# PoloWlg/Joint-Multimodal-Transformer-6th-ABAW

Measured on AMD Instinct MI355X. Metric: train windows/sec + CCC parity, B=64 T=300 A/V fusion, 1/2/4/8 MI355X, higher is better.
Workload: dtype bf16; 1 GPU; configs[2]: FcLayer(1024,512) + Two_transformers(TRANSFORMER,FC,H=1,L=1,vision_in_ft=2048) + 2x CCCLoss + SGD-nesterov; global_batch=64, per_gpu_batch=64, seq_len=300, D_a=1024, D_v=2048, parallelism=dp1

## Files before the change

### include/jmt.h

```cpp
#ifndef JMT_H_
#define JMT_H_

#include <stddef.h>
#include <stdint.h>

#ifdef __cplusplus
extern "C" {
#endif

#define JMT_ABI_VERSION 7

enum { JMT_F32 = 0, JMT_BF16 = 1, JMT_F16 = 2 };
enum { JMT_OK = 0, JMT_ERR_ARG = -1, JMT_ERR_HIP = -2, JMT_ERR_UNSUPPORTED = -3 };

int jmt_abi_version(void);
const char* jmt_last_error(void);
int jmt_kernel_count(void);
long long jmt_bounds_violations(int reset);

typedef struct jmt_gemm_desc {
  int ab_dtype, c_dtype, aux_dtype;
  int M, N, K;
  const void* a[8];
  const void* b[8];
// ... 58 lines not shown

int jmt_layernorm_fwd_grouped(int dt_in, int dt_out, int G, int64_t rows, int D, const void* x,
                              int64_t ldx, int64_t sx, const void* r, int64_t ldr, int64_t sr,
                              const float* const* gamma, const float* const* beta, float eps,
                              void* y, int64_t ldy, int64_t sy, float* mean, float* rstd,
                              void* stream);
int jmt_layernorm_bwd_grouped(int dt_in, int dt_dy, int dt_dx, int G, int64_t rows, int D,
                              const void* x, int64_t ldx, int64_t sx, const void* r, int64_t ldr,
                              int64_t sr, const void* dy, int64_t lddy, int64_t sdy,
                              const float* mean, const float* rstd, const float* const* gamma,
                              void* dx, int64_t lddx, int64_t sdx, float* const* dgamma,
                              float* const* dbeta, float* const* dsum, int beta_acc,
                              float* partials, void* stream);
int jmt_layernorm_bwd_grouped_blocks(int64_t rows);

int jmt_softmax_fwd(int p_dt, int64_t rows, int n, const float* s, int64_t lds, float scale,
                    void* p, int64_t ldp, void* stream);
int jmt_softmax_bwd(int p_dt, int ds_dt, int64_t rows, int n, const void* p, int64_t ldp,
                    const float* dp, int64_t lddp, float scale, void* ds, int64_t ldds,
                    void* stream);

int jmt_attn_supported(int dt, int dh);
int jmt_attn_fwd(int dt, int N, int H, int Lq, int Lk, int dh, const void* q, int64_t sq_l,
                 int64_t sq_n, const void* k, int64_t sk_l, int64_t sk_n, const void* v,
                 int64_t sv_l, int64_t sv_n, void* o, int64_t so_l, int64_t so_n, float scale,
                 float* lse, void* stream);
int jmt_attn_bwd(int dt, int N, int H, int Lq, int Lk, int dh, const void* go, int64_t sgo_l,
                 int64_t sgo_n, const void* o, int64_t so_l, int64_t so_n, const void* q,
                 int64_t sq_l, int64_t sq_n, const void* k, int64_t sk_l, int64_t sk_n,
                 const void* v, int64_t sv_l, int64_t sv_n, const float* lse, void* p_out,
                 void* ds_out, int64_t ldp, void* dq, int64_t sdq_l, int64_t sdq_n, float scale,
                 void* stream);

int jmt_attn_dkdv(int dt, int N, int H, int Lq, int Lk, int dh, const void* p, const void* ds,
                  int64_t ldp, const void* go, int64_t sgo_l, int64_t sgo_n, const void* q,
                  int64_t sq_l, int64_t sq_n, const void* k, int64_t sk_l, int64_t sk_n, void* dk,
                  int64_t sdk_l, int64_t sdk_n, void* dv, int64_t sdv_l, int64_t sdv_n, void* dq,
                  int64_t sdq_l, int64_t sdq_n, void* stream);

int jmt_attn_short_supported(int dt, int dh, int Lq, int Lk);
int jmt_attn_short_fwd(int dt, int N, int H, int Lq, int Lk, int dh, const void* q, int64_t sq_l,
                       int64_t sq_n, const void* k, int64_t sk_l, int64_t sk_n, const void* v,
                       int64_t sv_l, int64_t sv_n, void* o, int64_t so_l, int64_t so_n,
                       float scale, float* lse, void* stream);
int jmt_attn_short_bwd(int dt, int N, int H, int Lq, int Lk, int dh, const void* go,
                       int64_t sgo_l, int64_t sgo_n, const void* o, int64_t so_l, int64_t so_n,
                       const void* q, int64_t sq_l, int64_t sq_n, const void* k, int64_t sk_l,
                       int64_t sk_n, const void* v, int64_t sv_l, int64_t sv_n, const float* lse,
                       void* dq, int64_t sdq_l, int64_t sdq_n, void* dk, int64_t sdk_l,
                       int64_t sdk_n, void* dv, int64_t sdv_l, int64_t sdv_n, float scale,
                       void* stream);

int jmt_small_attn_fwd(int dt, int N, int H, int Lq, int Lk, int E, const void* q, int64_t sq_l,
                       int64_t sq_n, const void* k, int64_t sk_l, int64_t sk_n, const void* v,
                       int64_t sv_l, int64_t sv_n, void* o, int64_t so_l, int64_t so_n,
                       float scale, float* p_out, void* stream);
int jmt_small_attn_bwd(int dt, int N, int H, int Lq, int Lk, int E, const void* go,
                       int64_t sgo_l, int64_t sgo_n, const void* q, int64_t sq_l, int64_t sq_n,
                       const void* k, int64_t sk_l, int64_t sk_n, const void* v, int64_t sv_l,
                       int64_t sv_n, const float* p, void* dq, int64_t sdq_l, int64_t sdq_n,
                       void* dk, int64_t sdk_l, int64_t sdk_n, void* dv, int64_t sdv_l,
                       int64_t sdv_n, float scale, void* stream);

int jmt_colsum_blocks(int64_t rows);
int jmt_colsum(int dt, int64_t rows, int N, const void* dy, int64_t ld, float* db, int beta_acc,
               float* partials, void* stream);
// ... 86 lines not shown
```

### joint-multimodal-transformer-6th-abaw_amd/csrc/abi_check.cpp

```cpp
#include <stdio.h>
#include <string.h>

#include "../../include/jmt.h"

static int g_fail = 0;

static void expect_msg(const char* what, const char* needle) {
  const char* e = jmt_last_error();
  if (!e || !strstr(e, needle)) {
    fprintf(stderr, "FAIL %s: err='%s' lacks '%s'\n", what, e ? e : "(null)", needle);
    ++g_fail;
  }
}

static void expect_err(const char* what, int rc) {
  const char* e = jmt_last_error();
  const size_t n = e ? strnlen(e, 1024) : 0;
  if (rc >= 0 || n == 0 || n >= 512) {
    fprintf(stderr, "FAIL %s: rc=%d err='%s'\n", what, rc, e ? e : "(null)");
    ++g_fail;
  }
}

int main() {
// ... 93 lines not shown
  }

  expect_err("l2norm_fwd null", jmt_l2norm_fwd(JMT_BF16, JMT_BF16, 8, 512, nullptr, 512, nullptr,
                                               512, fnull, 1e-12f, nullptr));
  expect_err("layernorm_fwd dtype", jmt_layernorm_fwd(9, JMT_BF16, 8, 512, misal, 512, nullptr, 0,
                                                      fnull, fnull, 1e-5f, misal, 512, fnull,
                                                      fnull, nullptr));
  expect_err("softmax_fwd null", jmt_softmax_fwd(JMT_BF16, 8, 300, nullptr, 304, 1.f, nullptr, 304,
                                                 nullptr));
  expect_err("colsum null", jmt_colsum(JMT_BF16, 64, 512, nullptr, 512, fnull, 0, fnull, nullptr));
  expect_err("copy2d dtype", jmt_copy2d(5, 6, 4, 4, misal, 4, 1, misal, 4, 1, 0, nullptr));

  expect_err("attn_fwd head dim", jmt_attn_fwd(JMT_BF16, 2, 1, 300, 300, 64, misal, 512, 512,
                                               misal, 512, 512, misal, 512, 512, misal, 512, 512,
                                               0.1f, fnull, nullptr));
  expect_err("attn_fwd misaligned", jmt_attn_fwd(JMT_BF16, 2, 1, 300, 300, 512, misal, 512, 512,
                                                 misal, 512, 512, misal, 512, 512, misal, 512,
                                                 512, 0.1f, fnull, nullptr));
  expect_err("attn_bwd sizes", jmt_attn_bwd(JMT_BF16, -1, 1, 300, 300, 512, misal, 1, 1, misal, 1,
                                            1, misal, 1, 1, misal, 1, 1, misal, 1, 1, fnull,
                                            misal, misal, 8, misal, 1, 1, 0.1f, nullptr));
  expect_err("attn_dkdv ldp", jmt_attn_dkdv(JMT_BF16, 2, 1, 300, 300, 512, misal, misal, 320,
                                           misal, 512, 512, misal, 512, 512, nullptr, 0, 0,
                                           misal, 512, 512, misal, 512, 512, nullptr, 0, 0,
                                           nullptr));
  expect_err("attn_dkdv head dim", jmt_attn_dkdv(JMT_BF16, 2, 1, 300, 300, 64, misal, misal, 384,
                                                 misal, 512, 512, misal, 512, 512, nullptr, 0, 0,
                                                 misal, 512, 512, misal, 512, 512, nullptr, 0,
                                                 0, nullptr));
  expect_err("attn_dkdv dq misaligned", jmt_attn_dkdv(JMT_BF16, 2, 1, 300, 300, 512, algn, algn,
                                                      384, algn, 512, 512, algn, 512, 512, misal,
                                                      512, 512, algn, 512, 512, algn, 512, 512,
                                                      misal, 512, 512, nullptr));
  expect_err("attn_bwd pds ldp", jmt_attn_bwd(JMT_BF16, 2, 1, 300, 300, 512, algn, 512, 512,
                                              algn, 512, 512, algn, 512, 512, algn, 512, 512,
                                              algn, 512, 512, fnull, algn, algn, 300, nullptr,
                                              0, 0, 0.1f, nullptr));
  expect_err("small_attn_fwd null", jmt_small_attn_fwd(JMT_BF16, 4, 1, 6, 6, 512, nullptr, 512,
                                                       512, nullptr, 512, 512, nullptr, 512, 512,
                                                       nullptr, 512, 512, 0.1f, fnull, nullptr));

  expect_err("ccc_stats kind", jmt_ccc_stats(3, JMT_F32, 10, 1, misal, fnull, 0.f, -1.f, 1.f,
                                             nullptr, nullptr));
  expect_err("ccc_stats bins", jmt_ccc_stats(0, JMT_F32, 10, 100, misal, fnull, 0.f, -1.f, 1.f,
                                             (double*)buf, nullptr));
  expect_err("ccc_finish null", jmt_ccc_finish(0, 0, nullptr, 1, 1e-8f, fnull, nullptr, nullptr));
  expect_err("ccc_finish_add null", jmt_ccc_finish_add(0, 1, nullptr, 1, 1e-8f, fnull, fnull,
                                                       nullptr, nullptr));
  expect_err("ce_stats bins", jmt_ce_stats(JMT_F32, 10, 1, misal, fnull, -1.f, 1.f, fnull,
                                           (double*)buf, nullptr));
  expect_err("ce_bwd null", jmt_ce_bwd(JMT_F32, 10, 5, nullptr, fnull, -1.f, 1.f, fnull, nullptr,
                                       fnull, nullptr, nullptr));
  expect_err("ce_labels null", jmt_ce_labels(10, 5, fnull, -1.f, 1.f, nullptr, nullptr));
  expect_err("mask_indices null", jmt_mask_indices(10, fnull, -5.f, nullptr, nullptr, nullptr));

  expect_err("sgd null", jmt_sgd_step(10, fnull, fnull, fnull, 0.1f, 0.9f, 0.f, 0.f, 1, 1, 1.f,
                                      nullptr, JMT_BF16, nullptr));
  expect_err("sgd_zero null", jmt_sgd_step_zero(10, fnull, nullptr, fnull, 0.1f, 0.9f, 0.f, 0.f,
                                                1, 1, 1.f, nullptr, JMT_BF16, nullptr));
  expect_err("sgd_amp_zero null", jmt_sgd_step_amp_zero(10, fnull, fnull, fnull, 0.1f, 0.9f,
                                                        0.f, 0.f, 1, 1, nullptr, nullptr,
                                                        JMT_BF16, nullptr));
  float* fal = (float*)algn;
  expect_err("opt_tick null state", jmt_opt_tick(nullptr, 0.9, 0.999, nullptr, nullptr));
  expect_msg("opt_tick null state", "null state");
  expect_err("opt_tick beta", jmt_opt_tick(fal, 1.0, 0.999, nullptr, nullptr));
// ... 54 lines not shown
```

### joint-multimodal-transformer-6th-abaw_amd/csrc/attn_dkdv.hip

```cpp
#include "attn_common.h"

namespace jmt {

constexpr int DK_KT = 128;
constexpr int DK_QC = 32;
constexpr int DK_PROW = 2 * DK_KT;
constexpr int DK_IMG = DK_QC * AT_ROWB;
constexpr int DK_PIMG = DK_QC * DK_PROW;
constexpr int DK_STAGE = DK_IMG + DK_PIMG;
#ifndef JMT_DKDV_NS
#define JMT_DKDV_NS 4
#endif
constexpr int DK_NS = JMT_DKDV_NS;
constexpr int DK_LDS = DK_NS * DK_STAGE;
static_assert(DK_NS >= 2 && DK_NS <= 4, "2-4 stages (the wait table covers 0-2 later stages)");
constexpr int DK_NDMA = DK_QC / 8 + 1;
constexpr int DK_NST = 16;

struct AttnDkdvArgs {
  const void* p;
  const void* ds;
  const void* go;
  const void* q;
  const void* k;
  void* dk;
  void* dv;
  void* dq;
  int64_t ldp, sgo_l, sgo_n, sq_l, sq_n, sk_l, sk_n, sdk_l, sdk_n, sdv_l, sdv_n, sdq_l, sdq_n;
  int Lq, Lk, H, nkt, nqd, ipn, nitems;
};

__device__ __forceinline__ int pimg_off(int r, int c) {
  return r * DK_PROW + ((c ^ ((r & 7) << 1)) << 4);
}

__device__ __forceinline__ int qimg_off(int r, int c) {
  return r * 64 + ((c ^ ((r >> 2) & 3)) << 4);
}

struct DkItem {
  int nh, n, hd, role, k0, nch;
};
__device__ __forceinline__ DkItem dk_decode(const AttnDkdvArgs& a, int it) {
  DkItem d;
  d.nh = it / a.ipn;
  const int r = it - d.nh * a.ipn;
  if (r < 2 * a.nkt) {
    d.role = r >= a.nkt;
    d.k0 = (r - d.role * a.nkt) * DK_KT;
    d.nch = (a.Lq + DK_QC - 1) / DK_QC;
  } else {
    d.role = 2;
    d.k0 = (r - 2 * a.nkt) * DK_KT;
    d.nch = (a.Lk + DK_QC - 1) / DK_QC;
  }
  d.n = d.nh / a.H;
  d.hd = d.nh - d.n * a.H;
  return d;
}

template <typename T>
__device__ __forceinline__ void dkdv_stage(char* st, const AttnDkdvArgs& a, const DkItem& d,
                                           int q0) {
  const int lane = threadIdx.x & 63;
  const int wu = __builtin_amdgcn_readfirstlane(threadIdx.x >> 6);
  if (d.role == 2) {
    const char* kb = (const char*)((const T*)a.k + (int64_t)d.n * a.sk_n + d.hd * AT_DH);
    const int ldk = (int)(a.sk_l * (int64_t)sizeof(T));
#pragma unroll
    for (int i = 0; i < DK_QC / 8; ++i) {
      const int r = wu * (DK_QC / 8) + i;
      const int src = min(q0 + r, a.Lk - 1);
      const unsigned off = (unsigned)(lane ^ ((r & 7) << 1)) << 4;
      glds16_asm(kb + (unsigned)(src * ldk) + off, st + r * AT_ROWB);
    }
    const int r = 16 * wu + (lane >> 2);
    const int c = (lane & 3) ^ ((r >> 2) & 3);
    const int src_row = min(d.k0 + r, a.Lq - 1);
    JMT_DCHECK(src_row >= 0 && q0 + 8 * c + 8 <= a.ldp);
    const char* pb = (const char*)((const T*)a.ds + (int64_t)d.nh * a.Lq * a.ldp);
    glds16_asm(pb + (unsigned)(((q0 >> 5) * a.Lq + src_row) * 64) + 16 * c,
               st + DK_IMG + wu * 1024);
    return;
  }
  const char* rb;
  int ldb;
  if (d.role == 0) {
    rb = (const char*)((const T*)a.go + (int64_t)d.n * a.sgo_n + d.hd * AT_DH);
    ldb = (int)(a.sgo_l * (int64_t)sizeof(T));
  } else {
    rb = (const char*)((const T*)a.q + (int64_t)d.n * a.sq_n + d.hd * AT_DH);
    ldb = (int)(a.sq_l * (int64_t)sizeof(T));
  }
#pragma unroll
  for (int i = 0; i < DK_QC / 8; ++i) {
    const int r = wu * (DK_QC / 8) + i;
    const int src = min(q0 + r, a.Lq - 1);
    const unsigned off = (unsigned)(lane ^ ((r & 7) << 1)) << 4;
    glds16_asm(rb + (unsigned)(src * ldb) + off, st + r * AT_ROWB);
  }
  const int r = 4 * wu + (lane >> 4);
  const int cs = (lane & 15) ^ ((r & 7) << 1);
  const int src_row = min(q0 + r, a.Lq - 1);
  JMT_DCHECK(src_row >= 0 && d.k0 + 8 * cs + 8 <= a.ldp);
  if (a.dq) {
    const char* pb = (const char*)((const T*)(d.role == 0 ? a.p : a.ds) +
                                   (int64_t)d.nh * a.Lq * a.ldp);
    glds16_asm(pb + (unsigned)((((d.k0 >> 5) + (cs >> 2)) * a.Lq + src_row) * 64) +
                   16 * (cs & 3),
               st + DK_IMG + wu * 1024);
    return;
  }
  const char* pb = (const char*)((const T*)(d.role == 0 ? a.p : a.ds) +
                                 (int64_t)d.nh * a.Lq * a.ldp + d.k0);
  glds16_asm(pb + (unsigned)(src_row * (int)(a.ldp * sizeof(T))) + 16 * cs,
             st + DK_IMG + wu * 1024);
}

template <int S>
__device__ __forceinline__ void dkdv_wait_s(int stores) {
  switch (stores) {
    case 0: wait_vmcnt<S * DK_NDMA>(); break;
    case 1: wait_vmcnt<S * DK_NDMA + DK_NST>(); break;
    case 2: wait_vmcnt<S * DK_NDMA + 2 * DK_NST>(); break;
    default: wait_vmcnt<S * DK_NDMA + 3 * DK_NST>(); break;
  }
}
__device__ __forceinline__ void dkdv_wait(int stages, int stores) {
  if (stages == 0) dkdv_wait_s<0>(stores);
  else if (stages == 1) dkdv_wait_s<1>(stores);
  else dkdv_wait_s<2>(stores);
}

template <typename T>
__global__ __launch_bounds__(512, 2) void attn_dkdv_kernel(AttnDkdvArgs a) {
  typedef typename Frag16<T>::t F;
  typedef typename Frag16<T>::h Hf;
  typedef unsigned u32x4 __attribute__((ext_vector_type(4)));
  extern __shared__ __attribute__((aligned(16))) char smem[];
  const int lane = threadIdx.x & 63, w = threadIdx.x >> 6;
  const int g = lane >> 4, li = lane & 15;
  int item, iend, istride;
  item_range(a.nitems, item, iend, istride);
  if (item >= iend) return;

  int tb[4], pb[8];
#pragma unroll
  for (int t = 0; t < 4; ++t) tb[t] = tr_base(4 * (w & 1) + t, li, g, 0) + 256 * (w >> 1);
#pragma unroll
  for (int kg = 0; kg < 8; ++kg)
    pb[kg] = pimg_off(4 * g + (li >> 2), 2 * kg + ((li & 3) >> 1)) + 8 * (li & 1);
  const int qb0 = qimg_off(li, g >> 1) + 8 * (g & 1);
  const int qb1 = qimg_off(li, 2 + (g >> 1)) + 8 * (g & 1);

  int is_item = item, is_c = 0;
  DkItem is_d = dk_decode(a, item);
  bool is_ok = true;
  int is_buf = 0;
  unsigned after = 0;
  int inflight = 0;
  auto issue = [&]() {
    if (is_ok) {
      dkdv_stage<T>(smem + is_buf * DK_STAGE, a, is_d, DK_QC * is_c);
      after &= ~(15u << (4 * is_buf));
      ++inflight;
      if (++is_c == is_d.nch) {
        is_c = 0;
        is_item += istride;
        is_ok = is_item < iend;
        if (is_ok) is_d = dk_decode(a, is_item);
      }
    }
    is_buf = is_buf == DK_NS - 1 ? 0 : is_buf + 1;
  };
  for (int i = 0; i < DK_NS - 1; ++i) issue();
  int buf = 0;

  while (true) {
    const DkItem d = dk_decode(a, item);
    const bool more = item + istride < iend;
    f32x4 acc[8][4];
#pragma unroll
    for (int kg = 0; kg < 8; ++kg)
#pragma unroll
      for (int t = 0; t < 4; ++t) acc[kg][t] = f32x4{0.f, 0.f, 0.f, 0.f};

    for (int c = 0; c < d.nch; ++c) {
      const char* cur = smem + buf * DK_STAGE;
      dkdv_wait(inflight - 1, (after >> (4 * buf)) & 15);
      --inflight;
      lds_barrier();
      issue();
      F kf[8];
      const int c0 = DK_QC * c;
      const int clen = d.role == 2 ? a.Lk : a.Lq;
      if (d.role != 2) {
#pragma unroll
        for (int kg = 0; kg < 8; ++kg) {
          const Hf lo = tr_read<Hf>(cur + DK_IMG + pb[kg]);
          const Hf hi = tr_read<Hf>(cur + DK_IMG + pb[kg] + 16 * DK_PROW);
          kf[kg] = __builtin_shufflevector(lo, hi, 0, 1, 2, 3, 4, 5, 6, 7);
        }
      } else {
#pragma unroll
        for (int qg = 0; qg < 8; ++qg) {
          const Hf lo = *(const Hf*)(cur + DK_IMG + qb0 + 1024 * qg);
          const Hf hi = *(const Hf*)(cur + DK_IMG + qb1 + 1024 * qg);
          kf[qg] = __builtin_shufflevector(lo, hi, 0, 1, 2, 3, 4, 5, 6, 7);
        }
      }
      if (c0 + DK_QC > clen) {
#pragma unroll
        for (int e = 0; e < 8; ++e) {
          const bool in = c0 + 16 * (e >> 2) + 4 * g + (e & 3) < clen;
#pragma unroll
          for (int kg = 0; kg < 8; ++kg) kf[kg][e] = in ? kf[kg][e] : from_f<T>(0.f);
        }
      }
      F df[4];
#pragma unroll
      for (int t = 0; t < 4; ++t) {
        const Hf lo = tr_read<Hf>(cur + tb[t]);
        const Hf hi = tr_read<Hf>(cur + tb[t] + 16 * AT_ROWB);
        df[t] = __builtin_shufflevector(lo, hi, 0, 1, 2, 3, 4, 5, 6, 7);
      }
#pragma unroll
      for (int t = 0; t < 4; ++t)
#pragma unroll
        for (int kg = 0; kg < 8; ++kg) acc[kg][t] = mfma16(df[t], kf[kg], acc[kg][t]);
      buf = buf == DK_NS - 1 ? 0 : buf + 1;
    }

    {
      T* ob = d.role == 0 ? (T*)a.dv + (int64_t)d.n * a.sdv_n
            : d.role == 1 ? (T*)a.dk + (int64_t)d.n * a.sdk_n : (T*)a.dq + (int64_t)d.n * a.sdq_n;
      const int64_t sl = d.role == 0 ? a.sdv_l : d.role == 1 ? a.sdk_l : a.sdq_l;
      ob += (int64_t)d.hd * AT_DH + (int64_t)d.k0 * sl;
      const uint64_t ba = (uint64_t)(uintptr_t)ob;
      const uint32_t blo = __builtin_amdgcn_readfirstlane((uint32_t)ba);
      const uint32_t bhi = __builtin_amdgcn_readfirstlane((uint32_t)(ba >> 32));
      const int nrows = min(DK_KT, (d.role == 2 ? a.Lq : a.Lk) - d.k0);
      const int bytes = __builtin_amdgcn_readfirstlane((int)(nrows * sl * (int64_t)sizeof(T)));
      const auto rsrc = __builtin_amdgcn_make_buffer_rsrc(
          (void*)(((uint64_t)bhi << 32) | blo), 0, bytes, 0x00020000);
      const int sl32 = (int)sl;
#pragma unroll
      for (int kg = 0; kg < 8; ++kg) {
#pragma unroll
        for (int jp = 0; jp < 2; ++jp) {
          uint32_t pk[2][2];
#pragma unroll
          for (int hh = 0; hh < 2; ++hh)
#pragma unroll
            for (int qq = 0; qq < 2; ++qq) {
              T two[2] = {from_f<T>(acc[kg][2 * jp + hh][2 * qq]),
                          from_f<T>(acc[kg][2 * jp + hh][2 * qq + 1])};
              pk[hh][qq] = *(const uint32_t*)two;
            }
          const auto r0 = __builtin_amdgcn_permlane16_swap(pk[0][0], pk[1][0], false, false);
          const auto r1 = __builtin_amdgcn_permlane16_swap(pk[0][1], pk[1][1], false, false);
          const int col = 64 * w + 16 * (2 * jp + (g & 1)) + 8 * (g >> 1);
          const u32x4 v = {r0[0], r1[0], r0[1], r1[1]};
          const int off = ((16 * kg + li) * sl32 + col) * (int)sizeof(T);
          __builtin_amdgcn_raw_buffer_store_b128(v, rsrc, off, 0, 0);
        }
      }
    }
    after += 0x1111;
    if (!more) break;
    item += istride;
  }
  wait_vmcnt<0>();
}

static int dkdv_grid(int nitems) {
  static int ncu = 0;
  if (ncu == 0) {
    int dev = 0, v = 0;
    if (hipGetDevice(&dev) != hipSuccess ||
        hipDeviceGetAttribute(&v, hipDeviceAttributeMultiprocessorCount, dev) != hipSuccess || v < 8)
      v = 8;
    ncu = v / 8 * 8;
  }
  return nitems > ncu ? ncu : nitems;
}

}

using namespace jmt;

extern "C" int jmt_attn_dkdv(int dt, int N, int H, int Lq, int Lk, int dh, const void* p,
                             const void* ds, int64_t ldp, const void* go, int64_t sgo_l,
                             int64_t sgo_n, const void* q, int64_t sq_l, int64_t sq_n,
                             const void* k, int64_t sk_l, int64_t sk_n, void* dk, int64_t sdk_l,
                             int64_t sdk_n, void* dv, int64_t sdv_l, int64_t sdv_n, void* dq,
                             int64_t sdq_l, int64_t sdq_n, void* stream) {
  if (N == 0 || Lk == 0) return JMT_OK;
  if (!((dt == JMT_BF16 || dt == JMT_F16) && dh == AT_DH))
    return set_error(JMT_ERR_UNSUPPORTED, "jmt_attn_dkdv: dtype %d / head dim %d not supported",
                     dt, dh);
  JMT_CHECK_ARG(N > 0 && H > 0 && Lq > 0 && Lk > 0, "jmt_attn_dkdv: bad sizes");
  const void* ptrs[] = {p, ds, go, q, dk, dv};
  for (int i = 0; i < 6; ++i)
    JMT_CHECK_ARG(ptrs[i] != nullptr && ((uintptr_t)ptrs[i] & 15) == 0,
                  "jmt_attn_dkdv: operand %d null or not 16-B aligned", i);
  const int64_t strides[] = {ldp, sgo_l, sgo_n, sq_l, sq_n, sdk_l, sdk_n, sdv_l, sdv_n};
  for (int i = 0; i < 9; ++i)
    JMT_CHECK_ARG(strides[i] % 8 == 0, "jmt_attn_dkdv: stride %d not a multiple of 8", i);
  const int nkt = (Lk + DK_KT - 1) / DK_KT;
  JMT_CHECK_ARG(ldp >= (int64_t)nkt * DK_KT,
                "jmt_attn_dkdv: ldp must cover 128-key tiles (>= %d)", nkt * DK_KT);
  JMT_CHECK_ARG(sdk_l >= H * AT_DH && sdv_l >= H * AT_DH &&
                    (int64_t)DK_KT * sdk_l * 2 < (1LL << 31) &&
                    (int64_t)DK_KT * sdv_l * 2 < (1LL << 31),
                "jmt_attn_dkdv: dK / dV row stride out of range");
  const int nqd = dq ? (Lq + DK_KT - 1) / DK_KT : 0;
  if (dq) {
    JMT_CHECK_ARG(k != nullptr && ((uintptr_t)k & 15) == 0 && ((uintptr_t)dq & 15) == 0 &&
                      sk_l % 8 == 0 && sk_n % 8 == 0 && sdq_l % 8 == 0 && sdq_n % 8 == 0,
                  "jmt_attn_dkdv: k / dq null, misaligned or strides not multiples of 8");
    JMT_CHECK_ARG(sdq_l >= H * AT_DH && (int64_t)DK_KT * sdq_l * 2 < (1LL << 31) &&
                      (int64_t)Lk * sk_l * 2 < (1LL << 31),
                  "jmt_attn_dkdv: dQ / K row stride out of range");
  }
  JMT_CHECK_ARG((int64_t)N * H * (2 * nkt + nqd) < (1LL << 31), "jmt_attn_dkdv: too many items");
  JMT_CHECK_ARG((int64_t)Lq * sgo_l * 2 < (1LL << 31) && (int64_t)Lq * sq_l * 2 < (1LL << 31) &&
                    (int64_t)Lq * ldp * 2 < (1LL << 31),
                "jmt_attn_dkdv: Lq rows of dO / Q / P exceed 2 GiB");
  AttnDkdvArgs a = {};
  a.p = p; a.ds = ds; a.go = go; a.q = q; a.k = k; a.dk = dk; a.dv = dv; a.dq = dq;
  a.ldp = ldp; a.sgo_l = sgo_l; a.sgo_n = sgo_n; a.sq_l = sq_l; a.sq_n = sq_n;
  a.sk_l = sk_l; a.sk_n = sk_n;
  a.sdk_l = sdk_l; a.sdk_n = sdk_n; a.sdv_l = sdv_l; a.sdv_n = sdv_n;
  a.sdq_l = sdq_l; a.sdq_n = sdq_n;
  a.Lq = Lq; a.Lk = Lk; a.H = H; a.nkt = nkt; a.nqd = nqd; a.ipn = 2 * nkt + nqd;
  a.nitems = N * H * a.ipn;
  const dim3 grid(dkdv_grid(a.nitems));
  hipStream_t st = as_stream(stream);
  if (dt == JMT_BF16) {
    static bool once = ((void)hipFuncSetAttribute((const void*)attn_dkdv_kernel<__bf16>,
                                            hipFuncAttributeMaxDynamicSharedMemorySize, DK_LDS),
                        true);
    (void)once;
    hipLaunchKernelGGL((attn_dkdv_kernel<__bf16>), grid, dim3(512), (size_t)DK_LDS, st, a);
  } else {
    static bool once = ((void)hipFuncSetAttribute((const void*)attn_dkdv_kernel<_Float16>,
                                            hipFuncAttributeMaxDynamicSharedMemorySize, DK_LDS),
                        true);
    (void)once;
    hipLaunchKernelGGL((attn_dkdv_kernel<_Float16>), grid, dim3(512), (size_t)DK_LDS, st, a);
  }
  JMT_LAUNCH_CHECK("jmt_attn_dkdv");
  return JMT_OK;
}
```

### joint-multimodal-transformer-6th-abaw_amd/jmt/_lib.py

```python
from __future__ import annotations

import ctypes as C
import os

_HERE = os.path.dirname(os.path.abspath(__file__))
LIB_PATH = os.environ.get("JMT_LIB") or os.path.join(_HERE, "libjmt_hip.so")

F32, BF16, F16 = 0, 1, 2
OK, ERR_ARG, ERR_HIP, ERR_UNSUPPORTED = 0, -1, -2, -3

c_i64 = C.c_int64
c_vp = C.c_void_p
c_int = C.c_int
c_f = C.c_float
c_fp = C.POINTER(C.c_float)


class GemmDesc(C.Structure):
    _fields_ = [
        ("ab_dtype", c_int), ("c_dtype", c_int), ("aux_dtype", c_int),
        ("M", c_int), ("N", c_int), ("K", c_int),
        ("a", c_vp * 8), ("b", c_vp * 8), ("c", c_vp * 8),
        ("n_a", c_int), ("n_b", c_int), ("n_c", c_int),
        ("a_mode", c_int), ("b_mode", c_int), ("c_mode", c_int),
# ... 39 lines not shown
                                  c_vp, c_vp]),
    "jmt_layernorm_bwd_dsum": (c_int, [c_int, c_int, c_int, c_i64, c_int, c_vp, c_i64, c_vp,
                                       c_i64, c_vp, c_i64, c_vp, c_vp, c_vp, c_vp, c_i64, c_vp,
                                       c_vp, c_vp, c_int, c_vp, c_vp]),
    "jmt_layernorm_fwd_grouped": (c_int, [c_int, c_int, c_int, c_i64, c_int, c_vp, c_i64, c_i64,
                                          c_vp, c_i64, c_i64, c_vp, c_vp, c_f, c_vp, c_i64, c_i64,
                                          c_vp, c_vp, c_vp]),
    "jmt_layernorm_bwd_grouped": (c_int, [c_int, c_int, c_int, c_int, c_i64, c_int, c_vp, c_i64,
                                          c_i64, c_vp, c_i64, c_i64, c_vp, c_i64, c_i64, c_vp,
                                          c_vp, c_vp, c_vp, c_i64, c_i64, c_vp, c_vp, c_vp, c_int,
                                          c_vp, c_vp]),
    "jmt_softmax_fwd": (c_int, [c_int, c_i64, c_int, c_vp, c_i64, c_f, c_vp, c_i64, c_vp]),
    "jmt_softmax_bwd": (c_int, [c_int, c_int, c_i64, c_int, c_vp, c_i64, c_vp, c_i64, c_f, c_vp,
                                c_i64, c_vp]),
    "jmt_attn_supported": (c_int, [c_int, c_int]),
    "jmt_attn_fwd": (c_int, [c_int, c_int, c_int, c_int, c_int, c_int, c_vp, c_i64, c_i64, c_vp,
                             c_i64, c_i64, c_vp, c_i64, c_i64, c_vp, c_i64, c_i64, c_f, c_vp,
                             c_vp]),
    "jmt_attn_set_fwd_rows": (c_int, [c_int]),
    "jmt_attn_bwd": (c_int, [c_int, c_int, c_int, c_int, c_int, c_int, c_vp, c_i64, c_i64, c_vp,
                             c_i64, c_i64, c_vp, c_i64, c_i64, c_vp, c_i64, c_i64, c_vp, c_i64,
                             c_i64, c_vp, c_vp, c_vp, c_i64, c_vp, c_i64, c_i64, c_f, c_vp]),
    "jmt_attn_short_supported": (c_int, [c_int, c_int, c_int, c_int]),
    "jmt_attn_short_fwd": (c_int, [c_int, c_int, c_int, c_int, c_int, c_int, c_vp, c_i64, c_i64,
                                   c_vp, c_i64, c_i64, c_vp, c_i64, c_i64, c_vp, c_i64, c_i64,
                                   c_f, c_vp, c_vp]),
    "jmt_attn_short_bwd": (c_int, [c_int, c_int, c_int, c_int, c_int, c_int, c_vp, c_i64, c_i64,
                                   c_vp, c_i64, c_i64, c_vp, c_i64, c_i64, c_vp, c_i64, c_i64,
                                   c_vp, c_i64, c_i64, c_vp, c_vp, c_i64, c_i64, c_vp, c_i64,
                                   c_i64, c_vp, c_i64, c_i64, c_f, c_vp]),
    "jmt_attn_dkdv": (c_int, [c_int, c_int, c_int, c_int, c_int, c_int, c_vp, c_vp, c_i64, c_vp,
                              c_i64, c_i64, c_vp, c_i64, c_i64, c_vp, c_i64, c_i64, c_vp, c_i64,
                              c_i64, c_vp, c_i64, c_i64, c_vp, c_i64, c_i64, c_vp]),
    "jmt_noop": (c_int, [c_vp]),
    "jmt_small_attn_fwd": (c_int, [c_int, c_int, c_int, c_int, c_int, c_int, c_vp, c_i64, c_i64,
                                   c_vp, c_i64, c_i64, c_vp, c_i64, c_i64, c_vp, c_i64, c_i64,
                                   c_f, c_vp, c_vp]),
    "jmt_small_attn_bwd": (c_int, [c_int, c_int, c_int, c_int, c_int, c_int, c_vp, c_i64, c_i64,
                                   c_vp, c_i64, c_i64, c_vp, c_i64, c_i64, c_vp, c_i64, c_i64,
                                   c_vp, c_vp, c_i64, c_i64, c_vp, c_i64, c_i64, c_vp, c_i64,
                                   c_i64, c_f, c_vp]),
    "jmt_colsum_blocks": (c_int, [c_i64]),
    "jmt_layernorm_bwd_grouped_blocks": (c_int, [c_i64]),
    "jmt_colsum": (c_int, [c_int, c_i64, c_int, c_vp, c_i64, c_vp, c_int, c_vp, c_vp]),
    "jmt_colsum_grouped": (c_int, [c_int, c_int, c_i64, c_int, c_vp, c_i64, c_i64, c_vp, c_int,
                                   c_vp, c_vp]),
    "jmt_copy2d": (c_int, [c_int, c_int, c_i64, c_i64, c_vp, c_i64, c_i64, c_vp, c_i64, c_i64,
                           c_int, c_vp]),
    "jmt_ccc_stats": (c_int, [c_int, c_int, c_i64, c_int, c_vp, c_vp, c_f, c_f, c_f, c_vp, c_vp]),
    "jmt_ccc_finish": (c_int, [c_int, c_int, c_vp, c_i64, c_f, c_vp, c_vp, c_vp]),
    "jmt_ccc_finish_add": (c_int, [c_int, c_int, c_vp, c_i64, c_f, c_vp, c_vp, c_vp, c_vp]),
    "jmt_ccc_bwd": (c_int, [c_int, c_int, c_i64, c_int, c_vp, c_vp, c_f, c_f, c_f, c_vp, c_vp,
                            c_vp, c_vp]),
    "jmt_mask_indices": (c_int, [c_i64, c_vp, c_f, c_vp, c_vp, c_vp]),
    "jmt_vp_scatter": (c_int, [c_i64] + [c_vp] * 9 + [c_f, c_i64] + [c_vp] * 6),
    "jmt_vp_smooth": (c_int, [c_i64, c_int, c_vp, c_vp, c_vp, c_int, c_vp, c_vp]),
    "jmt_head_fwd": (c_int, [c_int, c_int, c_i64, c_int, c_int, c_vp, c_i64, c_vp, c_vp, c_vp,
                             c_vp, c_vp, c_vp, c_i64, c_vp]),
    "jmt_head_bwd": (c_int, [c_int, c_int, c_i64, c_int, c_int, c_vp, c_i64, c_vp, c_vp, c_vp,
                             c_vp, c_i64, c_vp, c_i64, c_vp, c_vp, c_vp, c_vp, c_vp, c_vp]),
    "jmt_head_bwd_workspace_bytes": (C.c_size_t, [c_i64]),
    "jmt_ce_stats": (c_int, [c_int, c_i64, c_int, c_vp, c_vp, c_f, c_f, c_vp, c_vp, c_vp]),
    "jmt_ce_finish": (c_int, [c_int, c_vp, c_vp, c_vp, c_vp]),
    "jmt_ce_bwd": (c_int, [c_int, c_i64, c_int, c_vp, c_vp, c_f, c_f, c_vp, c_vp, c_vp, c_vp,
                           c_vp]),
    "jmt_ce_labels": (c_int, [c_i64, c_int, c_vp, c_f, c_f, c_vp, c_vp]),
# ... 64 lines not shown
```

Before: 16510 windows/s.

## Add 160-row key tile variant for attention dK/dV/dQ kernel with cost-based selection

Templates the dK/dV/dQ backward kernel on the number of 16-row key groups and adds a 160-row tile path (10 groups, 3 stages) with its own tile-major P/dS DMA staging, swizzle and k-group blocking. A host-side cost model picks 160 rows when it gives less padded work for the given Lq/Lk. For T=300, two 160-row tiles replace three 128-row tiles, so less padded work is done. The cost is higher register pressure and fewer pipeline stages in the new variant, plus a new requirement that ldp be a multiple of 32 when dQ is produced.

```diff
diff --git a/include/jmt.h b/include/jmt.h
--- a/include/jmt.h
+++ b/include/jmt.h
@@ -114,6 +114,8 @@
                  void* ds_out, int64_t ldp, void* dq, int64_t sdq_l, int64_t sdq_n, float scale,
                  void* stream);
 
+int jmt_attn_dkdv_plan(int Lq, int Lk, int H, int64_t sdk_l, int64_t sdv_l, int64_t sdq_l,
+                       int has_dq);
 int jmt_attn_dkdv(int dt, int N, int H, int Lq, int Lk, int dh, const void* p, const void* ds,
                   int64_t ldp, const void* go, int64_t sgo_l, int64_t sgo_n, const void* q,
                   int64_t sq_l, int64_t sq_n, const void* k, int64_t sk_l, int64_t sk_n, void* dk,
diff --git a/joint-multimodal-transformer-6th-abaw_amd/csrc/abi_check.cpp b/joint-multimodal-transformer-6th-abaw_amd/csrc/abi_check.cpp
--- a/joint-multimodal-transformer-6th-abaw_amd/csrc/abi_check.cpp
+++ b/joint-multimodal-transformer-6th-abaw_amd/csrc/abi_check.cpp
@@ -149,6 +149,16 @@
                                                       384, algn, 512, 512, algn, 512, 512, misal,
                                                       512, 512, algn, 512, 512, algn, 512, 512,
                                                       misal, 512, 512, nullptr));
+  expect_err("attn_dkdv dq ldp % 32", jmt_attn_dkdv(JMT_BF16, 2, 1, 300, 300, 512, algn, algn,
+                                                    392, algn, 512, 512, algn, 512, 512, algn,
+                                                    512, 512, algn, 512, 512, algn, 512, 512,
+                                                    algn, 512, 512, nullptr));
+  if (jmt_attn_dkdv_plan(300, 300, 1, 512, 512, 512, 1) != 160 ||
+      jmt_attn_dkdv_plan(300, 300, 1, 512, 512, 512, 0) != 128 ||
+      jmt_attn_dkdv_plan(256, 256, 1, 512, 512, 512, 1) != 128) {
+    fprintf(stderr, "FAIL attn_dkdv_plan\n");
+    ++g_fail;
+  }
   expect_err("attn_bwd pds ldp", jmt_attn_bwd(JMT_BF16, 2, 1, 300, 300, 512, algn, 512, 512,
                                               algn, 512, 512, algn, 512, 512, algn, 512, 512,
                                               algn, 512, 512, fnull, algn, algn, 300, nullptr,
diff --git a/joint-multimodal-transformer-6th-abaw_amd/csrc/attn_dkdv.hip b/joint-multimodal-transformer-6th-abaw_amd/csrc/attn_dkdv.hip
--- a/joint-multimodal-transformer-6th-abaw_amd/csrc/attn_dkdv.hip
+++ b/joint-multimodal-transformer-6th-abaw_amd/csrc/attn_dkdv.hip
@@ -2,20 +2,30 @@
 
 namespace jmt {
 
-constexpr int DK_KT = 128;
 constexpr int DK_QC = 32;
-constexpr int DK_PROW = 2 * DK_KT;
 constexpr int DK_IMG = DK_QC * AT_ROWB;
-constexpr int DK_PIMG = DK_QC * DK_PROW;
-constexpr int DK_STAGE = DK_IMG + DK_PIMG;
 #ifndef JMT_DKDV_NS
 #define JMT_DKDV_NS 4
 #endif
-constexpr int DK_NS = JMT_DKDV_NS;
-constexpr int DK_LDS = DK_NS * DK_STAGE;
-static_assert(DK_NS >= 2 && DK_NS <= 4, "2-4 stages (the wait table covers 0-2 later stages)");
-constexpr int DK_NDMA = DK_QC / 8 + 1;
-constexpr int DK_NST = 16;
+
+template <int NKG>
+struct DkGeo {
+  static constexpr int KT = 16 * NKG;
+  static constexpr int PROW = 2 * KT;
+  static constexpr int PIMG = DK_QC * PROW;
+  static constexpr int STAGE = DK_IMG + PIMG;
+  static constexpr int NS = NKG == 8 ? JMT_DKDV_NS : 3;
+  static constexpr int LDS = NS * STAGE;
+  static constexpr int NPD = (PIMG / 1024 + 7) / 8;
+  static constexpr int PLANES = PIMG / 16 / 8 / NPD;
+  static constexpr int NDMA = DK_QC / 8 + NPD;
+  static constexpr int NST = 2 * NKG;
+  static_assert(NKG == 8 || NKG == 10, "128- or 160-row items");
+  static_assert(NS >= 2 && NS <= 4, "2-4 stages (the wait table covers 0-2 later stages)");
+  static_assert(LDS <= 160 * 1024, "stages exceed the LDS");
+  static_assert(8 * NPD * PLANES * 16 == PIMG && PLANES <= 64, "P / dS DMA split");
+  static_assert((NS - 2) * NDMA + (NS - 1) * NST < 64, "vmcnt range");
+};
 
 struct AttnDkdvArgs {
   const void* p;
@@ -31,7 +41,11 @@
 };
 
 __device__ __forceinline__ int pimg_off(int r, int c) {
-  return r * DK_PROW + ((c ^ ((r & 7) << 1)) << 4);
+  return r * DkGeo<8>::PROW + ((c ^ ((r & 7) << 1)) << 4);
+}
+
+__device__ __forceinline__ int simg_off(int r, int c) {
+  return r * 64 + ((c ^ ((r >> 1) & 2)) << 4);
 }
 
 __device__ __forceinline__ int qimg_off(int r, int c) {
@@ -41,17 +55,18 @@
 struct DkItem {
   int nh, n, hd, role, k0, nch;
 };
+template <int KT>
 __device__ __forceinline__ DkItem dk_decode(const AttnDkdvArgs& a, int it) {
   DkItem d;
   d.nh = it / a.ipn;
   const int r = it - d.nh * a.ipn;
   if (r < 2 * a.nkt) {
     d.role = r >= a.nkt;
-    d.k0 = (r - d.role * a.nkt) * DK_KT;
+    d.k0 = (r - d.role * a.nkt) * KT;
     d.nch = (a.Lq + DK_QC - 1) / DK_QC;
   } else {
     d.role = 2;
-    d.k0 = (r - 2 * a.nkt) * DK_KT;
+    d.k0 = (r - 2 * a.nkt) * KT;
     d.nch = (a.Lk + DK_QC - 1) / DK_QC;
   }
   d.n = d.nh / a.H;
@@ -117,26 +132,93 @@
              st + DK_IMG + wu * 1024);
 }
 
-template <int S>
+template <typename T>
+__device__ __forceinline__ void dkdv_stage160(uint32_t st, const AttnDkdvArgs& a, const DkItem& d,
+                                              int q0) {
+  typedef DkGeo<10> G;
+  const int lane = threadIdx.x & 63;
+  const int wu = __builtin_amdgcn_readfirstlane(threadIdx.x >> 6);
+  const char* rb;
+  int ldb, clen;
+  if (d.role == 0) {
+    rb = (const char*)((const T*)a.go + (int64_t)d.n * a.sgo_n + d.hd * AT_DH);
+    ldb = (int)(a.sgo_l * (int64_t)sizeof(T));
+    clen = a.Lq;
+  } else if (d.role == 1) {
+    rb = (const char*)((const T*)a.q + (int64_t)d.n * a.sq_n + d.hd * AT_DH);
+    ldb = (int)(a.sq_l * (int64_t)sizeof(T));
+    clen = a.Lq;
+  } else {
+    rb = (const char*)((const T*)a.k + (int64_t)d.n * a.sk_n + d.hd * AT_DH);
+    ldb = (int)(a.sk_l * (int64_t)sizeof(T));
+    clen = a.Lk;
+  }
+#pragma unroll
+  for (int i = 0; i < DK_QC / 8; ++i) {
+    const int r = wu * (DK_QC / 8) + i;
+    const int src = min(q0 + r, clen - 1);
+    JMT_DCHECK(src >= 0 && src < clen);
+    const unsigned off = (unsigned)(lane ^ ((r & 7) << 1)) << 4;
+    glds16_sv(rb + (unsigned)(src * ldb), off, st + r * AT_ROWB);
+  }
+  const char* pb = (const char*)((const T*)(d.role == 0 ? a.p : a.ds) +
+                                 (int64_t)d.nh * a.Lq * a.ldp);
+  const int ntile = (int)(a.ldp >> 5);
+  if (lane < G::PLANES) {
+#pragma unroll
+    for (int j = 0; j < G::NPD; ++j) {
+      const int b0 = (wu * G::NPD + j) * (16 * G::PLANES);
+      const int b = b0 + 16 * lane;
+      const int pc = (b >> 4) & 3;
+      int tile, row, c;
+      if (d.role == 2) {
+        const int r = b >> 6;
+        c = pc ^ ((r >> 2) & 3);
+        tile = q0 >> 5;
+        row = min(d.k0 + r, a.Lq - 1);
+      } else {
+        const int r = (b >> 6) & 31;
+        c = pc ^ ((r >> 1) & 2);
+        tile = min((d.k0 >> 5) + (b >> 11), ntile - 1);
+        row = min(q0 + r, a.Lq - 1);
+      }
+      JMT_DCHECK(row >= 0 && tile >= 0 && tile < ntile);
+      glds16_sv(pb, (unsigned)((tile * a.Lq + row) * 64 + 16 * c), st + DK_IMG + b0);
+    }
+  }
+}
+
+template <int NKG, int S>
 __device__ __forceinline__ void dkdv_wait_s(int stores) {
-  switch (stores) {
-    case 0: wait_vmcnt<S * DK_NDMA>(); break;
-    case 1: wait_vmcnt<S * DK_NDMA + DK_NST>(); break;
-    case 2: wait_vmcnt<S * DK_NDMA + 2 * DK_NST>(); break;
-    default: wait_vmcnt<S * DK_NDMA + 3 * DK_NST>(); break;
-  }
-}
+  typedef DkGeo<NKG> G;
+  if constexpr (S <= G::NS - 2) {
+    if (stores == 0) wait_vmcnt<S * G::NDMA>();
+    else if (stores == 1 || G::NS == 2) wait_vmcnt<S * G::NDMA + G::NST>();
+    else if constexpr (G::NS >= 3) {
+      if (stores == 2 || G::NS == 3) wait_vmcnt<S * G::NDMA + 2 * G::NST>();
+      else if constexpr (G::NS >= 4) wait_vmcnt<S * G::NDMA + 3 * G::NST>();
+    }
+  } else {
+    wait_vmcnt<0>();
+  }
+}
+template <int NKG>
 __device__ __forceinline__ void dkdv_wait(int stages, int stores) {
-  if (stages == 0) dkdv_wait_s<0>(stores);
-  else if (stages == 1) dkdv_wait_s<1>(stores);
-  else dkdv_wait_s<2>(stores);
-}
-
-template <typename T>
+  if (stages == 0) dkdv_wait_s<NKG, 0>(stores);
+  else if (stages == 1) dkdv_wait_s<NKG, 1>(stores);
+  else dkdv_wait_s<NKG, 2>(stores);
+}
+
+#define DK_NO_MERGE() asm volatile("" ::: "memory")
+
+template <typename T, int NKG>
 __global__ __launch_bounds__(512, 2) void attn_dkdv_kernel(AttnDkdvArgs a) {
   typedef typename Frag16<T>::t F;
   typedef typename Frag16<T>::h Hf;
   typedef unsigned u32x4 __attribute__((ext_vector_type(4)));
+  typedef DkGeo<NKG> G;
+  constexpr int KT = G::KT, NS = G::NS, STAGE = G::STAGE;
+  constexpr int KB = NKG == 8 ? 8 : 5;
   extern __shared__ __attribute__((aligned(16))) char smem[];
   const int lane = threadIdx.x & 63, w = threadIdx.x >> 6;
   const int g = lane >> 4, li = lane & 15;
@@ -144,91 +226,125 @@
   item_range(a.nitems, item, iend, istride);
   if (item >= iend) return;
 
-  int tb[4], pb[8];
-#pragma unroll
-  for (int t = 0; t < 4; ++t) tb[t] = tr_base(4 * (w & 1) + t, li, g, 0) + 256 * (w >> 1);
-#pragma unroll
-  for (int kg = 0; kg < 8; ++kg)
-    pb[kg] = pimg_off(4 * g + (li >> 2), 2 * kg + ((li & 3) >> 1)) + 8 * (li & 1);
+  int tb[NKG == 8 ? 4 : 1], pb[NKG == 8 ? 8 : 1];
+  if constexpr (NKG == 8) {
+#pragma unroll
+    for (int t = 0; t < 4; ++t) tb[t] = tr_base(4 * (w & 1) + t, li, g, 0) + 256 * (w >> 1);
+#pragma unroll
+    for (int kg = 0; kg < 8; ++kg)
+      pb[kg] = pimg_off(4 * g + (li >> 2), 2 * kg + ((li & 3) >> 1)) + 8 * (li & 1);
+  } else {
+    tb[0] = tr_base(4 * (w & 1), li, g, 0) + 256 * (w >> 1);
+    pb[0] = simg_off(4 * g + (li >> 2), (li & 3) >> 1) + 8 * (li & 1);
+  }
+  auto lane_base = [](int base, int bits) __attribute__((always_inline)) {
+#if !defined(__OPTIMIZE__)
+    return base ^ bits;
+#else
+    int r;
+    asm volatile("v_xor_b32 %0, %2, %1" : "=v"(r) : "v"(base), "i"(bits));
+    return r;
+#endif
+  };
   const int qb0 = qimg_off(li, g >> 1) + 8 * (g & 1);
-  const int qb1 = qimg_off(li, 2 + (g >> 1)) + 8 * (g & 1);
+  const int qb1 = NKG == 8 ? qimg_off(li, 2 + (g >> 1)) + 8 * (g & 1) : 0;
+  const uint32_t lbase = (uint32_t)(uintptr_t)(__attribute__((address_space(3))) char*)smem;
 
   int is_item = item, is_c = 0;
-  DkItem is_d = dk_decode(a, item);
+  DkItem is_d = dk_decode<KT>(a, item);
   bool is_ok = true;
   int is_buf = 0;
   unsigned after = 0;
   int inflight = 0;
   auto issue = [&]() {
     if (is_ok) {
-      dkdv_stage<T>(smem + is_buf * DK_STAGE, a, is_d, DK_QC * is_c);
+      if constexpr (NKG == 8) dkdv_stage<T>(smem + is_buf * STAGE, a, is_d, DK_QC * is_c);
+      else dkdv_stage160<T>(lbase + is_buf * STAGE, a, is_d, DK_QC * is_c);
       after &= ~(15u << (4 * is_buf));
       ++inflight;
       if (++is_c == is_d.nch) {
         is_c = 0;
         is_item += istride;
         is_ok = is_item < iend;
-        if (is_ok) is_d = dk_decode(a, is_item);
+        if (is_ok) is_d = dk_decode<KT>(a, is_item);
       }
     }
-    is_buf = is_buf == DK_NS - 1 ? 0 : is_buf + 1;
+    is_buf = is_buf == NS - 1 ? 0 : is_buf + 1;
   };
-  for (int i = 0; i < DK_NS - 1; ++i) issue();
+  for (int i = 0; i < NS - 1; ++i) issue();
   int buf = 0;
 
   while (true) {
-    const DkItem d = dk_decode(a, item);
+    const DkItem d = dk_decode<KT>(a, item);
     const bool more = item + istride < iend;
-    f32x4 acc[8][4];
-#pragma unroll
-    for (int kg = 0; kg < 8; ++kg)
+    f32x4 acc[NKG][4];
+#pragma unroll
+    for (int kg = 0; kg < NKG; ++kg)
 #pragma unroll
       for (int t = 0; t < 4; ++t) acc[kg][t] = f32x4{0.f, 0.f, 0.f, 0.f};
 
     for (int c = 0; c < d.nch; ++c) {
-      const char* cur = smem + buf * DK_STAGE;
-      dkdv_wait(inflight - 1, (after >> (4 * buf)) & 15);
+      const char* cur = smem + buf * STAGE;
+      dkdv_wait<NKG>(inflight - 1, (after >> (4 * buf)) & 15);
       --inflight;
       lds_barrier();
       issue();
-      F kf[8];
       const int c0 = DK_QC * c;
       const int clen = d.role == 2 ? a.Lk : a.Lq;
-      if (d.role != 2) {
-#pragma unroll
-        for (int kg = 0; kg < 8; ++kg) {
-          const Hf lo = tr_read<Hf>(cur + DK_IMG + pb[kg]);
-          const Hf hi = tr_read<Hf>(cur + DK_IMG + pb[kg] + 16 * DK_PROW);
-          kf[kg] = __builtin_shufflevector(lo, hi, 0, 1, 2, 3, 4, 5, 6, 7);
+      F df[4];
+#pragma unroll
+      for (int k0 = 0; k0 < NKG; k0 += KB) {
+        F kf[KB];
+        if (d.role != 2) {
+#pragma unroll
+          for (int j = 0; j < KB; ++j) {
+            const int kg = k0 + j;
+            const char* pa;
+            if constexpr (NKG == 8) pa = cur + DK_IMG + pb[kg];
+            else pa = cur + DK_IMG + lane_base(pb[0], (kg & 1) << 5) + 2048 * (kg >> 1);
+            const Hf lo = tr_read<Hf>(pa);
+            const Hf hi = tr_read<Hf>(pa + (NKG == 8 ? 16 * G::PROW : 16 * 64));
+            kf[j] = __builtin_shufflevector(lo, hi, 0, 1, 2, 3, 4, 5, 6, 7);
+          }
+        } else {
+          const char* qa0 = cur + DK_IMG + qb0;
+          const char* qa1;
+          if constexpr (NKG == 8) qa1 = cur + DK_IMG + qb1;
+          else qa1 = cur + DK_IMG + lane_base(qb0, 32);
+#pragma unroll
+          for (int j = 0; j < KB; ++j) {
+            const Hf lo = *(const Hf*)(qa0 + 1024 * (k0 + j));
+            DK_NO_MERGE();
+            const Hf hi = *(const Hf*)(qa1 + 1024 * (k0 + j));
+            DK_NO_MERGE();
+            kf[j] = __builtin_shufflevector(lo, hi, 0, 1, 2, 3, 4, 5, 6, 7);
+          }
         }
-      } else {
-#pragma unroll
-        for (int qg = 0; qg < 8; ++qg) {
-          const Hf lo = *(const Hf*)(cur + DK_IMG + qb0 + 1024 * qg);
-          const Hf hi = *(const Hf*)(cur + DK_IMG + qb1 + 1024 * qg);
-          kf[qg] = __builtin_shufflevector(lo, hi, 0, 1, 2, 3, 4, 5, 6, 7);
+        if (c0 + DK_QC > clen) {
+#pragma unroll
+          for (int e = 0; e < 8; ++e) {
+            const bool in = c0 + 16 * (e >> 2) + 4 * g + (e & 3) < clen;
+#pragma unroll
+            for (int j = 0; j < KB; ++j) kf[j][e] = in ? kf[j][e] : from_f<T>(0.f);
+          }
         }
+        if (k0 == 0) {
+#pragma unroll
+          for (int t = 0; t < 4; ++t) {
+            const char* ta;
+            if constexpr (NKG == 8) ta = cur + tb[t];
+            else ta = cur + lane_base(tb[0], t << 5);
+            const Hf lo = tr_read<Hf>(ta);
+            const Hf hi = tr_read<Hf>(ta + 16 * AT_ROWB);
+            df[t] = __builtin_shufflevector(lo, hi, 0, 1, 2, 3, 4, 5, 6, 7);
+          }
+        }
+#pragma unroll
+        for (int t = 0; t < 4; ++t)
+#pragma unroll
+          for (int j = 0; j < KB; ++j) acc[k0 + j][t] = mfma16(df[t], kf[j], acc[k0 + j][t]);
       }
-      if (c0 + DK_QC > clen) {
-#pragma unroll
-        for (int e = 0; e < 8; ++e) {
-          const bool in = c0 + 16 * (e >> 2) + 4 * g + (e & 3) < clen;
-#pragma unroll
-          for (int kg = 0; kg < 8; ++kg) kf[kg][e] = in ? kf[kg][e] : from_f<T>(0.f);
-        }
-      }
-      F df[4];
-#pragma unroll
-      for (int t = 0; t < 4; ++t) {
-        const Hf lo = tr_read<Hf>(cur + tb[t]);
-        const Hf hi = tr_read<Hf>(cur + tb[t] + 16 * AT_ROWB);
-        df[t] = __builtin_shufflevector(lo, hi, 0, 1, 2, 3, 4, 5, 6, 7);
-      }
-#pragma unroll
-      for (int t = 0; t < 4; ++t)
-#pragma unroll
-        for (int kg = 0; kg < 8; ++kg) acc[kg][t] = mfma16(df[t], kf[kg], acc[kg][t]);
-      buf = buf == DK_NS - 1 ? 0 : buf + 1;
+      buf = buf == NS - 1 ? 0 : buf + 1;
     }
 
     {
@@ -239,13 +355,13 @@
       const uint64_t ba = (uint64_t)(uintptr_t)ob;
       const uint32_t blo = __builtin_amdgcn_readfirstlane((uint32_t)ba);
       const uint32_t bhi = __builtin_amdgcn_readfirstlane((uint32_t)(ba >> 32));
-      const int nrows = min(DK_KT, (d.role == 2 ? a.Lq : a.Lk) - d.k0);
+      const int nrows = min(KT, (d.role == 2 ? a.Lq : a.Lk) - d.k0);
       const int bytes = __builtin_amdgcn_readfirstlane((int)(nrows * sl * (int64_t)sizeof(T)));
       const auto rsrc = __builtin_amdgcn_make_buffer_rsrc(
           (void*)(((uint64_t)bhi << 32) | blo), 0, bytes, 0x00020000);
       const int sl32 = (int)sl;
 #pragma unroll
-      for (int kg = 0; kg < 8; ++kg) {
+      for (int kg = 0; kg < NKG; ++kg) {
 #pragma unroll
         for (int jp = 0; jp < 2; ++jp) {
           uint32_t pk[2][2];
@@ -285,9 +401,57 @@
   return nitems > ncu ? ncu : nitems;
 }
 
+static int64_t dkdv_cost(int Lq, int Lk, int KT) {
+  const auto cdiv = [](int x, int d) { return ((int64_t)x + d - 1) / d; };
+  return (2 * cdiv(Lk, KT) * cdiv(Lq, DK_QC) + cdiv(Lq, KT) * cdiv(Lk, DK_QC)) * KT;
+}
+
+static int g_dkdv_tile = -1;
+static int dkdv_tile_pref() {
+  static const int env = [] {
+    const char* e = getenv("JMT_ATTN_DKDV_KT");
+    const int v = e ? atoi(e) : 0;
+    return v == 128 || v == 160 ? v : 0;
+  }();
+  return g_dkdv_tile < 0 ? env : g_dkdv_tile;
+}
+
+static int dkdv_plan(int Lq, int Lk, int64_t sdk_l, int64_t sdv_l, int64_t sdq_l, bool has_dq) {
+  constexpr int64_t KT = DkGeo<10>::KT;
+  if (!has_dq || Lq <= 0 || Lk <= 0 || KT * sdk_l * 2 >= (1LL << 31) ||
+      KT * sdv_l * 2 >= (1LL << 31) || KT * sdq_l * 2 >= (1LL << 31))
+    return 128;
+  const int pref = dkdv_tile_pref();
+  if (pref) return pref;
+  return dkdv_cost(Lq, Lk, 160) < dkdv_cost(Lq, Lk, 128) ? 160 : 128;
+}
+
+template <typename T, int NKG>
+static void dkdv_launch(const AttnDkdvArgs& a, int grid, hipStream_t st) {
+  constexpr int lds = DkGeo<NKG>::LDS;
+  static bool once = ((void)hipFuncSetAttribute((const void*)attn_dkdv_kernel<T, NKG>,
+                                                hipFuncAttributeMaxDynamicSharedMemorySize, lds),
+                      true);
+  (void)once;
+  hipLaunchKernelGGL((attn_dkdv_kernel<T, NKG>), dim3(grid), dim3(512), (size_t)lds, st, a);
+}
+
 }
 
 using namespace jmt;
+
+extern "C" int jmt_attn_dkdv_set_tile(int kt) {
+  if (!(kt < 0 || kt == 0 || kt == 128 || kt == 160))
+    return set_error(JMT_ERR_ARG, "jmt_attn_dkdv_set_tile: %d is not 0, 128 or 160", kt);
+  g_dkdv_tile = kt < 0 ? -1 : kt;
+  return JMT_OK;
+}
+
+extern "C" int jmt_attn_dkdv_plan(int Lq, int Lk, int H, int64_t sdk_l, int64_t sdv_l,
+                                  int64_t sdq_l, int has_dq) {
+  (void)H;
+  return dkdv_plan(Lq, Lk, sdk_l, sdv_l, sdq_l, has_dq != 0);
+}
 
 extern "C" int jmt_attn_dkdv(int dt, int N, int H, int Lq, int Lk, int dh, const void* p,
                              const void* ds, int64_t ldp, const void* go, int64_t sgo_l,
@@ -295,6 +459,7 @@
                              const void* k, int64_t sk_l, int64_t sk_n, void* dk, int64_t sdk_l,
                              int64_t sdk_n, void* dv, int64_t sdv_l, int64_t sdv_n, void* dq,
                              int64_t sdq_l, int64_t sdq_n, void* stream) {
+  constexpr int DK_KT = DkGeo<8>::KT;
   if (N == 0 || Lk == 0) return JMT_OK;
   if (!((dt == JMT_BF16 || dt == JMT_F16) && dh == AT_DH))
     return set_error(JMT_ERR_UNSUPPORTED, "jmt_attn_dkdv: dtype %d / head dim %d not supported",
@@ -307,14 +472,13 @@
   const int64_t strides[] = {ldp, sgo_l, sgo_n, sq_l, sq_n, sdk_l, sdk_n, sdv_l, sdv_n};
   for (int i = 0; i < 9; ++i)
     JMT_CHECK_ARG(strides[i] % 8 == 0, "jmt_attn_dkdv: stride %d not a multiple of 8", i);
-  const int nkt = (Lk + DK_KT - 1) / DK_KT;
-  JMT_CHECK_ARG(ldp >= (int64_t)nkt * DK_KT,
-                "jmt_attn_dkdv: ldp must cover 128-key tiles (>= %d)", nkt * DK_KT);
+  JMT_CHECK_ARG(ldp >= (int64_t)((Lk + DK_KT - 1) / DK_KT) * DK_KT,
+                "jmt_attn_dkdv: ldp must cover 128-key tiles (>= %d)",
+                (Lk + DK_KT - 1) / DK_KT * DK_KT);
   JMT_CHECK_ARG(sdk_l >= H * AT_DH && sdv_l >= H * AT_DH &&
                     (int64_t)DK_KT * sdk_l * 2 < (1LL << 31) &&
                     (int64_t)DK_KT * sdv_l * 2 < (1LL << 31),
                 "jmt_attn_dkdv: dK / dV row stride out of range");
-  const int nqd = dq ? (Lq + DK_KT - 1) / DK_KT : 0;
   if (dq) {
     JMT_CHECK_ARG(k != nullptr && ((uintptr_t)k & 15) == 0 && ((uintptr_t)dq & 15) == 0 &&
                       sk_l % 8 == 0 && sk_n % 8 == 0 && sdq_l % 8 == 0 && sdq_n % 8 == 0,
@@ -322,7 +486,11 @@
     JMT_CHECK_ARG(sdq_l >= H * AT_DH && (int64_t)DK_KT * sdq_l * 2 < (1LL << 31) &&
                       (int64_t)Lk * sk_l * 2 < (1LL << 31),
                   "jmt_attn_dkdv: dQ / K row stride out of range");
-  }
+    JMT_CHECK_ARG(ldp % 32 == 0, "jmt_attn_dkdv: tile-major P / dS need ldp %% 32 == 0");
+  }
+  const int kt = dkdv_plan(Lq, Lk, sdk_l, sdv_l, dq ? sdq_l : 0, dq != nullptr);
+  const int nkt = (Lk + kt - 1) / kt;
+  const int nqd = dq ? (Lq + kt - 1) / kt : 0;
   JMT_CHECK_ARG((int64_t)N * H * (2 * nkt + nqd) < (1LL << 31), "jmt_attn_dkdv: too many items");
   JMT_CHECK_ARG((int64_t)Lq * sgo_l * 2 < (1LL << 31) && (int64_t)Lq * sq_l * 2 < (1LL << 31) &&
                     (int64_t)Lq * ldp * 2 < (1LL << 31),
@@ -335,20 +503,14 @@
   a.sdq_l = sdq_l; a.sdq_n = sdq_n;
   a.Lq = Lq; a.Lk = Lk; a.H = H; a.nkt = nkt; a.nqd = nqd; a.ipn = 2 * nkt + nqd;
   a.nitems = N * H * a.ipn;
-  const dim3 grid(dkdv_grid(a.nitems));
+  const int grid = dkdv_grid(a.nitems);
   hipStream_t st = as_stream(stream);
-  if (dt == JMT_BF16) {
-    static bool once = ((void)hipFuncSetAttribute((const void*)attn_dkdv_kernel<__bf16>,
-                                            hipFuncAttributeMaxDynamicSharedMemorySize, DK_LDS),
-                        true);
-    (void)once;
-    hipLaunchKernelGGL((attn_dkdv_kernel<__bf16>), grid, dim3(512), (size_t)DK_LDS, st, a);
+  if (kt == 160) {
+    if (dt == JMT_BF16) dkdv_launch<__bf16, 10>(a, grid, st);
+    else dkdv_launch<_Float16, 10>(a, grid, st);
   } else {
-    static bool once = ((void)hipFuncSetAttribute((const void*)attn_dkdv_kernel<_Float16>,
-                                            hipFuncAttributeMaxDynamicSharedMemorySize, DK_LDS),
-                        true);
-    (void)once;
-    hipLaunchKernelGGL((attn_dkdv_kernel<_Float16>), grid, dim3(512), (size_t)DK_LDS, st, a);
+    if (dt == JMT_BF16) dkdv_launch<__bf16, 8>(a, grid, st);
+    else dkdv_launch<_Float16, 8>(a, grid, st);
   }
   JMT_LAUNCH_CHECK("jmt_attn_dkdv");
   return JMT_OK;
diff --git a/joint-multimodal-transformer-6th-abaw_amd/jmt/_lib.py b/joint-multimodal-transformer-6th-abaw_amd/jmt/_lib.py
--- a/joint-multimodal-transformer-6th-abaw_amd/jmt/_lib.py
+++ b/joint-multimodal-transformer-6th-abaw_amd/jmt/_lib.py
@@ -95,6 +95,8 @@
     "jmt_attn_dkdv": (c_int, [c_int, c_int, c_int, c_int, c_int, c_int, c_vp, c_vp, c_i64, c_vp,
                               c_i64, c_i64, c_vp, c_i64, c_i64, c_vp, c_i64, c_i64, c_vp, c_i64,
                               c_i64, c_vp, c_i64, c_i64, c_vp, c_i64, c_i64, c_vp]),
+    "jmt_attn_dkdv_plan": (c_int, [c_int, c_int, c_int, c_i64, c_i64, c_i64, c_int]),
+    "jmt_attn_dkdv_set_tile": (c_int, [c_int]),
     "jmt_noop": (c_int, [c_vp]),
     "jmt_small_attn_fwd": (c_int, [c_int, c_int, c_int, c_int, c_int, c_int, c_vp, c_i64, c_i64,
                                    c_vp, c_i64, c_i64, c_vp, c_i64, c_i64, c_vp, c_i64, c_i64,
```

After: 16740 windows/s, median of 6. +1.4%, better.
